# DerEchteKarsten/RayTracer3

Measured on AMD Instinct MI355X. Metric: Mrays/s, higher is better.
Workload: dtype f32

## Files before the change

### raytracer3_amd/csrc/rt3_accel.hip

```cpp
#include <hip/hip_runtime.h>

#include <cmath>
#include <cstring>
#include <algorithm>
#include <chrono>
#include <string>
#include <vector>

#include "rt3_ctx.hpp"

using namespace rt3;

namespace rt3 {

void invalidate_accel(rt3_ctx* c) { c->accel.built = false; }
void mark_accel_stale(rt3_ctx* c) {
    if (c->accel.built) c->accel.stale = true;
}
int check_accel_current(rt3_ctx* c, const char* unbuilt) {
    if (!c || !c->accel.built) return fail(c, RT3_E_STATE, unbuilt);
    if (c->accel.stale) return fail(c, RT3_E_STATE, "vertices were updated since the acceleration structure was built: rt3_accel_refit or rt3_accel_build first");
    return RT3_OK;
}
std::pair<const rt3_instance*, size_t> placements(const rt3_ctx* c, rt3_instance& whole) {
// ... 432 lines not shown
            if (from[q] >= 0) {
                const TlMesh& om = tl.meshes[from[q]];
                meshes[q].n_nodes = om.n_nodes;
                meshes[q].depth = om.depth;
                memcpy(meshes[q].box, om.box, sizeof(om.box));
            } else {
                rc = tl_build_mesh(c, meshes[q], &built[q]);
                tl.n_built++;
            }
        }
        uint64_t nodes_total = head, tris_total = 0;
        for (auto& m : meshes) {
            m.node_off = (uint32_t)nodes_total;
            m.tri_off = (uint32_t)tris_total;
            nodes_total += m.n_nodes;
            tris_total += m.n_tris;
        }
        if (rc == RT3_OK && (nodes_total >= (1ull << 29) || tris_total > (1ull << 28)))
            rc = fail(c, RT3_E_UNSUPPORTED, "instance mode 1: the bottom trees exceed the 28-bit references");
        DevBuf<float4> nodes, tris;
        hipError_t e = hipSuccess;
        if (rc == RT3_OK) {
            e = nodes.alloc_bytes((size_t)nodes_total * 64);
            if (e == hipSuccess) e = tris.alloc_bytes((size_t)tris_total * 48 + 128);
            if (e == hipSuccess) e = hipMemsetAsync((char*)tris.get() + (size_t)tris_total * 48, 0, 128, c->stream);
            for (size_t q = 0; e == hipSuccess && q < meshes.size(); q++) {
                const TlMesh& m = meshes[q];
                if (from[q] >= 0) {
                    const TlMesh& om = tl.meshes[from[q]];
                    tlas_rebase_nodes(c->stream, c->accel.bvh.nodes.get() + 4 * (size_t)om.node_off, nodes.get() + 4 * (size_t)m.node_off, m.n_nodes, om.node_off,
                                      m.node_off, om.tri_off, m.tri_off);
                    e = hipMemcpyAsync(tris.get() + 3 * (size_t)m.tri_off, c->accel.bvh.tris.get() + 3 * (size_t)om.tri_off, (size_t)m.n_tris * 48, hipMemcpyDeviceToDevice,
                                       c->stream);
                } else {
                    tlas_rebase_nodes(c->stream, built[q].nodes.get(), nodes.get() + 4 * (size_t)m.node_off, m.n_nodes, 0u, m.node_off, 0u, m.tri_off);
                    e = hipMemcpyAsync(tris.get() + 3 * (size_t)m.tri_off, built[q].tris.get(), (size_t)m.n_tris * 48, hipMemcpyDeviceToDevice, c->stream);
                }
            }
            if (e == hipSuccess) e = hipGetLastError();
            if (e == hipSuccess) e = hipStreamSynchronize(c->stream);
            if (e != hipSuccess) rc = fail(c, RT3_E_HIP, std::string("two-level: bottom trees: ") + hipGetErrorString(e));
        }
        if (rc != RT3_OK) {
            free_accel(c);
            return rc;
        }
        c->accel.bvh.nodes = std::move(nodes);
        c->accel.bvh.tris = std::move(tris);
        tl.meshes = meshes;
        tl.head = head;
        tl.gen = c->scene.content_gen;
        tl.n_alloc_nodes = (uint32_t)nodes_total;
        tl.valid = true;
    }
    tl.inst = std::move(ii);
    tl.n_placed = n_ne;
    tl.top_cap = top_cap;
    return tl_records_and_top(c);
}
// ... 63 lines not shown
            return rc;
        }
    }
    if (int r = accel_finish(c, out_handle)) return r;
    c->prof.stats.accel_build_ms = std::chrono::duration<double, std::milli>(std::chrono::steady_clock::now() - t_build0).count();
    return RT3_OK;
}
int rt3_accel_info(rt3_ctx* c, uint32_t* n_nodes, uint32_t* n_tris, uint32_t* max_depth, uint32_t* node_bytes) {
    if (!c || !c->accel.built) return fail(c, RT3_E_STATE, "no acceleration structure built");
    if (n_nodes) *n_nodes = c->accel.bvh.n_nodes;
    if (n_tris) *n_tris = c->accel.bvh.n_tris;
    if (max_depth) *max_depth = c->accel.bvh.max_depth;
    if (node_bytes) *node_bytes = c->accel.bvh.node_bytes;
    return RT3_OK;
}
int rt3_accel_levels(rt3_ctx* c, uint32_t* n_meshes, uint32_t* n_meshes_built, uint32_t* n_top_nodes, uint64_t* accel_bytes) {
    if (!c || !c->accel.built) return fail(c, RT3_E_STATE, "no acceleration structure built");
    const bool two = c->accel.bvh.layout == kLayoutTwoLevel;
    if (n_meshes) *n_meshes = two ? c->accel.tl.n_meshes : 0u;
    if (n_meshes_built) *n_meshes_built = two ? c->accel.tl.n_built : 0u;
    if (n_top_nodes) *n_top_nodes = two ? c->accel.tl.n_top : 0u;
    if (accel_bytes) {
        const uint64_t nodes = !c->accel.bvh.nodes ? 0u : (two ? (uint64_t)c->accel.tl.n_alloc_nodes * 64u : (uint64_t)c->accel.bvh.n_nodes * c->accel.bvh.node_bytes);
        *accel_bytes = nodes + (!c->accel.bvh.tris ? 0u : (uint64_t)c->accel.bvh.n_tris * 48u) + (uint64_t)c->accel.bvh.n_top * 64u;
    }
    return RT3_OK;
}
int rt3_accel_download(rt3_ctx* c, void* nodes, size_t nodes_bytes, void* tris, size_t tris_bytes) {
    if (int r = check_accel_current(c, "no acceleration structure built")) return r;
    if (c->accel.bvh.layout == kLayoutTwoLevel) return fail(c, RT3_E_UNSUPPORTED, "accel_download: not for the two-level structure (RT3_OPT_INSTANCE_MODE 1)");
    if (nodes) {
        if (nodes_bytes != (size_t)c->accel.bvh.n_nodes * c->accel.bvh.node_bytes) return fail(c, RT3_E_INVALID, "nodes_bytes mismatch");
        if (nodes_bytes) HIPC(c, hipMemcpy(nodes, c->accel.bvh.nodes.get(), nodes_bytes, hipMemcpyDeviceToHost));
    }
    if (tris) {
        if (tris_bytes != (size_t)c->accel.bvh.n_tris * 48) return fail(c, RT3_E_INVALID, "tris_bytes mismatch");
        if (tris_bytes) HIPC(c, hipMemcpy(tris, c->accel.bvh.tris.get(), tris_bytes, hipMemcpyDeviceToHost));
    }
    return RT3_OK;
}
int rt3_accel_import(rt3_ctx* c, const void* nodes, size_t nodes_bytes, const void* tris, size_t tris_bytes) {
    if (!c || !nodes || !tris) return fail(c, RT3_E_INVALID, "accel_import: NULL argument");
    if (!c->accel.built) return fail(c, RT3_E_STATE, "accel_import: build the scene's own structure first (rt3_accel_build makes the shading records)");
    if (c->accel.bvh.layout == kLayoutTwoLevel) return fail(c, RT3_E_UNSUPPORTED, "accel_import: not for the two-level structure (RT3_OPT_INSTANCE_MODE 1)");
    if (c->accel.bvh.layout != kLayoutWide64Q) return fail(c, RT3_E_UNSUPPORTED, "accel_import: default node layout only");
    if (any_cutoff(c)) return fail(c, RT3_E_UNSUPPORTED, "accel_import: not for a scene with alpha-masked geometry (rt3_scene_set_alpha_cutoffs)");
    if (nodes_bytes == 0 || nodes_bytes % 64 || tris_bytes % 48 || nodes_bytes / 64 > 0x3FFFFFFFull) return fail(c, RT3_E_INVALID, "accel_import: sizes must be multiples of 64 / 48 bytes");
    const uint32_t nn = (uint32_t)(nodes_bytes / 64), nt = (uint32_t)(tris_bytes / 48);
    const uint32_t* w = static_cast<const uint32_t*>(nodes);
    const uint32_t* tw = static_cast<const uint32_t*>(tris);
    for (uint32_t k = 0; k < nt; k++)
        if (tw[12 * (size_t)k + 9] >= c->accel.n_flat_prims) return fail(c, RT3_E_INVALID, "accel_import: triangle record " + std::to_string(k) + " names a primitive the scene does not have");
    std::vector<uint8_t> seen(nn, 0);
    std::vector<std::pair<uint32_t, uint32_t>> st;
    st.emplace_back(0u, 1u);
    seen[0] = 1;
    uint32_t max_level = 1;
    while (!st.empty()) {
        const auto [node, level] = st.back();
        st.pop_back();
        max_level = level > max_level ? level : max_level;
        for (int k = 0; k < 4; k++) {
            const uint32_t ref = w[16 * (size_t)node + 10 + k];
            if (ref == 0xFFFFFFFFu) continue;
            if (ref & 0x80000000u) {
                const uint64_t first = ref & 0x0FFFFFFFu, cnt = ((ref >> 28) & 7u) + 1u;
                if (first + cnt > nt) return fail(c, RT3_E_INVALID, "accel_import: node " + std::to_string(node) + " references triangles beyond the array");
            } else {
                if (ref >= nn || seen[ref]) return fail(c, RT3_E_INVALID, "accel_import: node " + std::to_string(node) + " references a node out of range or reachable twice");
                seen[ref] = 1;
                st.emplace_back(ref, level + 1);
            }
        }
    }
    const uint32_t depth = max_level + 1;
    if (stack_entries(4, depth) > kMaxStack) return fail(c, RT3_E_DEPTH, "accel_import: the tree is deeper than the traversal stack supports");
    HIPC(c, hipSetDevice(c->device));
    HIPC(c, hipStreamSynchronize(c->stream));
    DevBuf<float4> d_nodes, d_tris;
    HIPC(c, d_nodes.alloc_bytes(nodes_bytes));
    hipError_t e = d_tris.alloc_bytes(tris_bytes + 128);
    if (e == hipSuccess) e = hipMemset(d_tris.get(), 0, tris_bytes + 128);
    if (e == hipSuccess) e = hipMemcpy(d_nodes.get(), nodes, nodes_bytes, hipMemcpyHostToDevice);
    if (e == hipSuccess && tris_bytes) e = hipMemcpy(d_tris.get(), tris, tris_bytes, hipMemcpyHostToDevice);
    if (e != hipSuccess) return fail(c, RT3_E_HIP, std::string("accel_import: ") + hipGetErrorString(e));
    c->accel.bvh.nodes = std::move(d_nodes);
    c->accel.bvh.tris = std::move(d_tris);
    c->accel.bvh.n_nodes = nn;
    c->accel.bvh.n_tris = nt;
    c->accel.bvh.max_depth = depth;
    c->accel.refit_planned = false;
    bump_stamp(c);
    e = lbvh_make_top(c->stream, c->accel.bvh.nodes.get(), nn, c->accel.bvh.top, &c->accel.bvh.n_top);
    if (e != hipSuccess) {
        invalidate_accel(c);
        return fail(c, RT3_E_HIP, std::string("accel_import: top-of-tree copy: ") + hipGetErrorString(e));
    }
    return RT3_OK;
}

struct RefitScratch {
    uint32_t* bounds;
    float *nbox, *tbox;
};
static int refit_scratch(rt3_ctx* c, size_t n_nodes, size_t n_tris, RefitScratch* s) {
    BufLayout plan;
    plan.add(&s->bounds, 6).add(&s->nbox, 6 * n_nodes).add(&s->tbox, 6 * n_tris);
// ... 96 lines not shown
```

### raytracer3_amd/csrc/rt3_internal.hpp

```cpp
#pragma once
#include <hip/hip_runtime.h>
#include <stddef.h>
#include <stdint.h>

#include <vector>

#include "rt3_device.hpp"

#define RT3_FLAG_NEE_SKY 1u
#define RT3_FLAG_BLUENOISE 2u
#define RT3_FLAG_SPECULAR 4u
#define RT3_FLAG_FACEFORWARD 8u
#define RT3_FLAG_PROBE_RADIANCE 16u
#define RT3_FLAG_NEE_EMISSIVE 32u

namespace rt3 {

constexpr int kExtendBlock = 256;
constexpr unsigned kExtendMaxBlocks = 2048;
constexpr int kLayoutBinary64 = 0;
constexpr int kLayoutWide128 = 1;
constexpr int kLayoutWide48Q = 3;
constexpr int kC48Stride = 3;
constexpr int kLayoutWide64Q = 2;
constexpr int kLayoutTwoLevel = 4;
constexpr uint32_t kMaxStack = 64;
constexpr uint32_t kTopCacheNodes = 128;
enum TotalsWord : int {
    kTotExtendNodes = 0,
    kTotExtendTris = 1,
    kTotShadowNodes = 2,
    kTotShadowTris = 3,
    kTotExtendLds = 4,
    kTotShadowLds = 5,
    kTotWords = 6
};

struct ShadeLaunch {
    GConstDev g;
    SceneDev sc;
    const uint32_t* pixels;
    const uint2* pixbn;
    uint32_t npix, width;
    FastDiv npix_div;
    uint32_t s0;
    uint32_t bounce;
    const uint4* gbuffer;
    const float* depth;
// ... 246 lines not shown
};
static_assert(sizeof(MotionPrevDev) == 64, "MotionPrev layout");
struct MotionDev {
    const float* verts;
    const uint32_t *indices, *prim_geom, *first_prim, *geom_slot;
    const FlatGeomDev* geoms;
    const MotionPrevDev* prev;
};
struct MotionLaunch {
    GConstDev g;
    MotionDev m;
    const uint32_t* pixels;
    uint32_t npix, width;
    const float* hits;
    void* out;
    const float4* prev_pos = nullptr;
};
void launch_motion(hipStream_t st, const MotionLaunch& L);
void launch_snapshot_positions(hipStream_t st, const float* verts, uint32_t first, uint32_t n, float4* prev_pos);
constexpr uint32_t kDeformChunk = 1024;
void launch_compare_positions(hipStream_t st, const float* verts, const float4* prev_pos, const uint4* chunks, uint32_t n_chunks, uint32_t* flags);

hipError_t lbvh_make_top(hipStream_t st, const float4* nodes, uint32_t n_nodes, DevBuf<float4>& top, uint32_t* n_top);

}
```

### raytracer3_amd/csrc/rt3_kernels.hip

```cpp
#include <hip/hip_fp16.h>
#include <hip/hip_runtime.h>

#include <type_traits>

#include "rt3_device.hpp"
#include "rt3_internal.hpp"

namespace rt3 {

constexpr int kLdsStack = 12;
constexpr uint32_t kTopFlag = 0x40000000u;
constexpr int kSpill = 64 - kLdsStack;
constexpr uint32_t kMaxSteps = 1u << 20;

constexpr uint32_t kEmptySlot = 0xFFFFFFFFu;
constexpr float kTopPadRel = 2.44140625e-4f;

struct Cand {
    float tn;
    uint32_t ref;
};
__device__ __forceinline__ void cswap(Cand& a, Cand& b) {
    bool sw = b.tn < a.tn;
    float ta = a.tn;
// ... 170 lines not shown
                r.sp = 0;
                r.index = idx;
                r.steps = 0u;
                r.cn = r.ct = r.cl = 0u;
                busy = true;
                const float kMaxF = 3.4028234663852886e38f;
                const bool finite_ray = fabsf(r.o.x) <= kMaxF && fabsf(r.o.y) <= kMaxF && fabsf(r.o.z) <= kMaxF && fabsf(r.d.x) <= kMaxF &&
                                        fabsf(r.d.y) <= kMaxF && fabsf(r.d.z) <= kMaxF;
                if (nodes == nullptr || !finite_ray) {
                    finish(r.index, r.best, 0u, 0u, 0u, r.pay0, r.pay1, r.pay2, r.pay3);
                    busy = false;
                }
            }
            const uint32_t taken = (uint32_t)__popcll(m_idle);
            pool_next = pool_next + taken < pool_end ? pool_next + taken : pool_end;
        }
        if (__ballot(busy) == 0ull && pool_next >= pool_end && queue_empty) break;
        if (busy) {
        const bool is_leaf = (r.cur & 0x80000000u) != 0u;
        const uint32_t first = r.cur & 0x0FFFFFFFu, cnt = ((r.cur >> 28) & 7u) + 1u;
        const bool cached = LAYOUT == kLayoutWide64Q && !is_leaf && (r.cur & kTopFlag) != 0u;
        const bool is_inst = TWO && is_leaf && !tl_bottom;
        const bool is_tri = is_leaf && !is_inst;
        const float4* p = is_tri ? tris + 3 * (size_t)(first + r.leaf_k)
                                 : nodes + (WIDE ? 8 : (C48 ? kC48Stride : 4)) * (size_t)(cached ? 0u : (is_inst ? first : r.cur));
        float4 q0, q1, q2, q3, q4, q5, q6, q7;
        if (LAYOUT == kLayoutWide64Q && cached) {
            const float4* t = top_lds + 4 * (r.cur & 0xFFFFu);
            q0 = t[0];
            q1 = t[1];
            q2 = t[2];
            q3 = t[3];
        } else {
            q0 = p[0];
            q1 = p[1];
            q2 = p[2];
            q3 = C48 ? make_float4(0.0f, 0.0f, 0.0f, 0.0f) : p[3];
        }
        if (WIDE) {
            q4 = p[4];
            q5 = p[5];
            q6 = p[6];
            q7 = p[7];
        }
        if (TWO && is_tri) {
            const float4* pm = nodes + 4 * (size_t)(tl_rec + 1u);
            q4 = pm[0];
// ... 1003 lines not shown
```

### raytracer3_amd/csrc/rt3_lbvh.hip

```cpp
#include <hip/hip_runtime.h>
#include <hipcub/hipcub.hpp>

#include <chrono>
#include <cstdio>
#include <cstdlib>
#include <vector>

#include "rt3_device.hpp"
#include "rt3_internal.hpp"
#include "rt3_bvh_device.hpp"

namespace rt3 {

__global__ void k_prim_geom(const uint32_t* first_prim, uint32_t n_geoms, uint32_t n, uint32_t* prim_geom) {
    for (uint32_t p = blockIdx.x * blockDim.x + threadIdx.x; p < n; p += gridDim.x * blockDim.x) {
        uint32_t lo = 0, hi = n_geoms;
        while (hi - lo > 1u) {
            uint32_t mid = (lo + hi) >> 1;
            if (first_prim[mid] <= p) lo = mid;
            else hi = mid;
        }
        prim_geom[p] = lo;
    }
}
// ... 85 lines not shown

__global__ void k_morton(const float* bmin, const float* bmax, const uint32_t* bounds, uint32_t n, uint64_t* keys, uint32_t* vals) {
    float cmin[3], cext[3];
#pragma unroll
    for (int k = 0; k < 3; k++) {
        cmin[k] = ordered_to_float(bounds[6 + k]);
        cext[k] = ordered_to_float(bounds[9 + k]) - cmin[k];
    }
    for (uint32_t i = blockIdx.x * blockDim.x + threadIdx.x; i < n; i += gridDim.x * blockDim.x) {
        uint32_t q[3];
#pragma unroll
        for (int k = 0; k < 3; k++) {
            float ce = (bmin[3 * (size_t)i + k] + bmax[3 * (size_t)i + k]) * 0.5f;
            float nrm = cext[k] > 0.0f ? (ce - cmin[k]) / cext[k] : 0.0f;
            q[k] = (uint32_t)fmin_sel(nrm * 2097152.0f, 2097151.0f);
        }
        keys[i] = (expand21(q[0]) << 2) | (expand21(q[1]) << 1) | expand21(q[2]);
        vals[i] = i;
    }
}

__global__ void k_leaves(const float* verts, const uint32_t* indices, const FlatGeomDev* geoms, const uint32_t* prim_geom,
                         const uint32_t* first_prim, const uint32_t* sorted_prim, const float* bmin, const float* bmax,
                         const uint32_t* bounds, uint32_t n, float4* tris, float* lmin, float* lmax, const uint2* geom_mask) {
    const float pad = leaf_pad(bounds);
    for (uint32_t k = blockIdx.x * blockDim.x + threadIdx.x; k < n; k += gridDim.x * blockDim.x) {
        uint32_t p = sorted_prim[k];
        V3 a, b, c;
        fetch_triangle(verts, indices, geoms, prim_geom, first_prim, p, a, b, c);
        tris[3 * (size_t)k + 0] = make_float4(a.x, a.y, a.z, b.x);
        tris[3 * (size_t)k + 1] = make_float4(b.y, b.z, c.x, c.y);
        const uint2 mk = geom_mask ? geom_mask[geoms[prim_geom[p]].geom] : make_uint2(0u, 0u);
        tris[3 * (size_t)k + 2] = make_float4(c.z, __uint_as_float(p), __uint_as_float(mk.x), __uint_as_float(mk.y));
#pragma unroll
        for (int j = 0; j < 3; j++) {
            lmin[3 * (size_t)k + j] = bmin[3 * (size_t)p + j] - pad;
            lmax[3 * (size_t)k + j] = bmax[3 * (size_t)p + j] + pad;
        }
    }
}

__device__ __forceinline__ int delta(const uint64_t* codes, int n, int i, int j) {
    if (j < 0 || j >= n) return -1;
    uint64_t a = codes[i], b = codes[j];
    if (a != b) return __clzll((long long)(a ^ b));
    return 64 + __clz((int)((uint32_t)i ^ (uint32_t)j));
}

__global__ void k_hierarchy(const uint64_t* codes, int n, uint32_t* left, uint32_t* right, uint32_t* parent_internal, uint32_t* parent_leaf,
                            uint32_t* range_lo, uint32_t* range_cnt) {
    for (int i = blockIdx.x * blockDim.x + threadIdx.x; i < n - 1; i += gridDim.x * blockDim.x) {
        int d = (delta(codes, n, i, i + 1) - delta(codes, n, i, i - 1)) >= 0 ? 1 : -1;
        int dmin = delta(codes, n, i, i - d);
        int lmax = 2;
        while (delta(codes, n, i, i + lmax * d) > dmin) lmax *= 2;
        int l = 0;
// ... 209 lines not shown
        }
    }
}
__device__ __forceinline__ uint32_t tree_position(uint32_t me_ref, uint32_t parent, const uint32_t* left, const uint32_t* right, const uint32_t* parent_internal,
                                                  const uint32_t* range_cnt) {
    uint32_t pos = 0;
    while (parent != 0xFFFFFFFFu) {
        if (right[parent] == me_ref) {
            const uint32_t l = left[parent];
            pos += (l & 0x80000000u) ? 1u : range_cnt[l];
        }
        me_ref = parent;
        parent = parent_internal[parent];
    }
    return pos;
}
__global__ void k_tree_order(const uint32_t* left, const uint32_t* right, const uint32_t* parent_internal, const uint32_t* parent_leaf, const uint32_t* range_cnt,
                             uint32_t n, uint32_t nn, uint32_t* newpos, uint32_t* range_lo) {
    for (uint32_t t = blockIdx.x * blockDim.x + threadIdx.x; t < n + nn; t += gridDim.x * blockDim.x) {
        if (t < n) newpos[t] = tree_position(0x80000000u | t, parent_leaf[t], left, right, parent_internal, range_cnt);
        else range_lo[t - n] = tree_position(t - n, parent_internal[t - n], left, right, parent_internal, range_cnt);
    }
}
__global__ void k_tree_reorder(const uint32_t* newpos, uint32_t n, uint32_t nn, const float4* tris_in, float4* tris_out, const float* lmin_in, const float* lmax_in,
                               float* lmin_out, float* lmax_out, uint32_t* left, uint32_t* right) {
    for (uint32_t t = blockIdx.x * blockDim.x + threadIdx.x; t < n + nn; t += gridDim.x * blockDim.x) {
        if (t < n) {
            const uint32_t p = newpos[t];
#pragma unroll
            for (int k = 0; k < 3; k++) tris_out[3 * (size_t)p + k] = tris_in[3 * (size_t)t + k];
#pragma unroll
            for (int j = 0; j < 3; j++) {
                lmin_out[3 * (size_t)p + j] = lmin_in[3 * (size_t)t + j];
                lmax_out[3 * (size_t)p + j] = lmax_in[3 * (size_t)t + j];
            }
        } else {
            const uint32_t i = t - n, l = left[i], r = right[i];
            if (l & 0x80000000u) left[i] = 0x80000000u | newpos[l & 0x7FFFFFFFu];
            if (r & 0x80000000u) right[i] = 0x80000000u | newpos[r & 0x7FFFFFFFu];
        }
    }
}

__device__ __forceinline__ uint32_t gather_slots(uint32_t i, const uint32_t* left, const uint32_t* right, const uint32_t* live,
                                                 const float* nbox, const uint32_t* dk, int wide, int collapse, uint32_t sl[4]) {
    uint32_t ns = 0;
    if (wide && collapse == 2) {
        uint32_t sn[8], sm[8];
        int sp = 0;
        const uint32_t k4 = dk[i] & 3u;
        sl[0] = sl[1] = sl[2] = sl[3] = 0xFFFFFFFFu;
        sn[sp] = right[i]; sm[sp++] = 4u - k4;
        sn[sp] = left[i]; sm[sp++] = k4;
// ... 163 lines not shown
__global__ void k_top_cache(const float4* __restrict__ nodes, uint32_t n_nodes, uint32_t* __restrict__ top_words , uint32_t* __restrict__ n_top_out) {
    if (blockIdx.x != 0 || threadIdx.x != 0) return;
    uint32_t queue[kTopCacheNodes];
    uint32_t head = 0, tail = 0;
    if (n_nodes) queue[tail++] = 0u;
    while (head < tail) {
        const uint32_t node = queue[head];
        const uint32_t* src = reinterpret_cast<const uint32_t*>(nodes + 4 * (size_t)node);
        uint32_t* dst = top_words + 16 * (size_t)head;
        for (int k = 0; k < 16; k++) dst[k] = src[k];
        for (int k = 0; k < 4; k++) {
            const uint32_t ref = src[10 + k];
            if (ref == 0xFFFFFFFFu || (ref & 0x80000000u)) continue;
            if (tail < kTopCacheNodes) {
                dst[10 + k] = 0x40000000u | tail;
                queue[tail++] = ref;
            }
        }
        head++;
    }
    *n_top_out = tail;
}

hipError_t lbvh_make_top(hipStream_t st, const float4* nodes, uint32_t n_nodes, DevBuf<float4>& top, uint32_t* n_top) {
    *n_top = 0;
    if (!top) {
        hipError_t e = top.alloc_bytes((size_t)kTopCacheNodes * 64);
        if (e != hipSuccess) return e;
    }
    DevBuf<uint32_t> d_ntop;
    hipError_t e = d_ntop.alloc_bytes(4);
    if (e != hipSuccess) return e;
    hipLaunchKernelGGL(k_top_cache, dim3(1), dim3(1), 0, st, nodes, n_nodes, (uint32_t*)top.get(), d_ntop.get());
    e = hipMemcpyAsync(n_top, d_ntop.get(), 4, hipMemcpyDeviceToHost, st);
    if (e == hipSuccess) e = hipStreamSynchronize(st);
    return e;
}

__global__ void k_single(const float* lmin, const float* lmax, int wide, int quant, float4* nodes) {
    const float inf = INFINITY;
    if (wide && quant) {
        float qmn[4][3], qmx[4][3];
        uint32_t qref[4] = {0x80000000u, 0, 0, 0};
        for (int j = 0; j < 3; j++) {
            qmn[0][j] = lmin[j];
            qmx[0][j] = lmax[j];
// ... 64 lines not shown
    const bool dp = collapse == 2;
    out->node_bytes = (wide && !quant) ? 128u : (quant == 2 ? 16u * kC48Stride : 64u);
    out->layout = !wide ? kLayoutBinary64 : (quant == 2 ? kLayoutWide48Q : (quant ? kLayoutWide64Q : kLayoutWide128));
    if (n == 0) return hipSuccess;
    const uint32_t nn = n > 1 ? n - 1 : 1;
    LbvhScratch s = {};
    {
        BufLayout plan;
        RT3_TRY(plan_scratch(st, n, quant, collapse, sah_top != 0, wide && quant == 1, plan, &s));
        RT3_TRY(scratch.grow_bytes(plan.bytes()));
        RT3_TRY(plan.carve(scratch));
        if (getenv("RT3_TRACE_BUILD"))
            fprintf(stderr, "rt3 build: %u triangles, scratch %zu bytes (radix sort %zu, scan %zu)\n", n, plan.bytes(), s.sort_bytes, s.scan_bytes);
    }
    const unsigned grid = (unsigned)(((uint64_t)n + 255) / 256 > 4096 ? 4096 : ((uint64_t)n + 255) / 256);
    uint32_t init_bounds[12];
    uint32_t tail[2] = {0, 0};
    for (int k = 0; k < 3; k++) {
        init_bounds[k] = 0xFFFFFFFFu;
        init_bounds[3 + k] = 0u;
        init_bounds[6 + k] = 0xFFFFFFFFu;
        init_bounds[9 + k] = 0u;
    }
    RT3_TRY(out->tris.alloc_bytes((size_t)n * 48 + 128));
    RT3_TRY(hipMemsetAsync((char*)out->tris.get() + (size_t)n * 48, 0, 128, st));
    RT3_TRY(hipMemcpyAsync(s.bounds, init_bounds, sizeof(init_bounds), hipMemcpyHostToDevice, st));
    RT3_TRY(hipMemsetAsync(s.arrive, 0, (size_t)nn * 4, st));
    RT3_TRY(hipMemsetAsync(s.levels, 0, 4, st));
    hipLaunchKernelGGL(k_prim_bounds, dim3(grid > 512 ? 512 : grid), dim3(256), 0, st, t.verts, t.indices, t.geoms, t.prim_geom, t.first_prim, n, s.bmin, s.bmax, s.bounds);
    hipLaunchKernelGGL(k_morton, dim3(grid), dim3(256), 0, st, s.bmin, s.bmax, s.bounds, n, s.keys_in, s.vals_in);
    RT3_TRY(hipcub::DeviceRadixSort::SortPairs(s.sort_tmp, s.sort_bytes, s.keys_in, s.keys_out, s.vals_in, s.vals_out, (int)n, 0, 63, st));
    hipLaunchKernelGGL(k_leaves, dim3(grid), dim3(256), 0, st, t.verts, t.indices, t.geoms, t.prim_geom, t.first_prim, s.vals_out, s.bmin, s.bmax, s.bounds, n,
                       s.tris_dp ? s.tris_dp : (s.tris_morton ? s.tris_morton : out->tris.get()), s.lmin, s.lmax, geom_mask);
    if (n == 1) {
        RT3_TRY(out->nodes.alloc_bytes(out->node_bytes));
        hipLaunchKernelGGL(k_single, dim3(1), dim3(1), 0, st, s.lmin, s.lmax, wide, quant, out->nodes.get());
        out->n_nodes = 1;
        out->max_depth = 2;
        RT3_TRY(hipGetLastError());
        RT3_TRY(hipStreamSynchronize(st));
    } else {
        hipLaunchKernelGGL(k_hierarchy, dim3(grid), dim3(256), 0, st, s.keys_out, (int)n, s.left, s.right, s.pint, s.pleaf, s.rlo, s.rcnt);
        const uint32_t T_sah = dp ? sah_top : (sah_top > leaf_max ? sah_top : leaf_max);
        const bool lite = sah_top && T_sah <= 64;
        if (lite) hipLaunchKernelGGL(k_refit_clusters, dim3(grid), dim3(256), 0, st, s.rlo, s.rcnt, s.lmin, s.lmax, nn, T_sah, s.nbox);
        else hipLaunchKernelGGL(k_refit, dim3(grid), dim3(256), 0, st, s.left, s.right, s.pint, s.pleaf, s.lmin, s.lmax, n, s.nbox, s.arrive);
        if (sah_top) {
            bool relinked = false;
            const auto t0 = std::chrono::steady_clock::now();
            RT3_TRY(sah_top_relink_gpu(st, nn, s.left, s.right, s.rcnt, s.pint, s.pleaf, s.lmin, s.lmax, s.nbox, T_sah, s.sah, &relinked));
            if (!relinked && lite) {
                RT3_TRY(hipMemsetAsync(s.arrive, 0, (size_t)nn * 4, st));
                hipLaunchKernelGGL(k_refit, dim3(grid), dim3(256), 0, st, s.left, s.right, s.pint, s.pleaf, s.lmin, s.lmax, n, s.nbox, s.arrive);
            }
            if (getenv("RT3_TRACE_BUILD")) {
                RT3_TRY(hipStreamSynchronize(st));
                fprintf(stderr, "rt3 build: device SAH top (incl. GPU LBVH drain) %.2f ms\n",
                        std::chrono::duration<double, std::milli>(std::chrono::steady_clock::now() - t0).count());
            }
        }
        const auto t3 = std::chrono::steady_clock::now();
        if (dp) {
            RT3_TRY(hipMemsetAsync(s.arrive, 0, (size_t)nn * 4, st));
            hipLaunchKernelGGL(k_dp_up, dim3(grid), dim3(256), 0, st, s.left, s.right, s.pint, s.pleaf, s.lmin, s.lmax, s.nbox, n, leaf_max, s.rcnt, s.dc, s.dk,
                               s.live, s.arrive);
            const unsigned g3 = (unsigned)(((uint64_t)n + nn + 255) / 256 > 4096 ? 4096 : ((uint64_t)n + nn + 255) / 256);
            hipLaunchKernelGGL(k_tree_order, dim3(g3), dim3(256), 0, st, s.left, s.right, s.pint, s.pleaf, s.rcnt, n, nn, s.newpos, s.rlo);
            float4* tris_to = quant == 2 ? s.tris_morton : out->tris.get();
            hipLaunchKernelGGL(k_tree_reorder, dim3(g3), dim3(256), 0, st, s.newpos, n, nn, s.tris_dp, tris_to, s.lmin, s.lmax, s.lmin2, s.lmax2, s.left, s.right);
            s.lmin = s.lmin2;
            s.lmax = s.lmax2;
        } else {
            hipLaunchKernelGGL(k_live_flags, dim3(grid), dim3(256), 0, st, s.rcnt, nn, leaf_max, s.live);
        }
        if (collapse) {
            const uint32_t root = 0, one = 1;
            const size_t n_cnt = (size_t)nn + 18;
            RT3_TRY(hipMemsetAsync(s.keep, 0, (size_t)nn * 4, st));
            RT3_TRY(hipMemsetAsync(s.fr_n, 0, n_cnt * 4, st));
            RT3_TRY(hipMemcpyAsync(s.fr_a, &root, 4, hipMemcpyHostToDevice, st));
            RT3_TRY(hipMemcpyAsync(s.fr_n, &one, 4, hipMemcpyHostToDevice, st));
            const unsigned g2 = (unsigned)((nn + 255) / 256 > 1024 ? 1024 : (nn + 255) / 256);
            uint32_t level = 0, last = 1, wide_levels = 0;
            while (last > 0 && level + 16 < n_cnt) {
                for (int burst = 0; burst < 16; burst++, level++) {
                    hipLaunchKernelGGL(k_wide_level, dim3(g2), dim3(256), 0, st, s.left, s.right, s.live, s.nbox, s.dk, collapse, s.fr_a, s.fr_n + level, s.keep,
                                       s.fr_b, s.fr_n + level + 1);
                    std::swap(s.fr_a, s.fr_b);
                }
                RT3_TRY(hipMemcpyAsync(&last, s.fr_n + level, 4, hipMemcpyDeviceToHost, st));
                RT3_TRY(hipStreamSynchronize(st));
            }
// ... 41 lines not shown
```

### raytracer3_amd/csrc/rt3_refit.hip

```cpp
#include <hip/hip_runtime.h>

#include "rt3_bvh_device.hpp"
#include "rt3_internal.hpp"

namespace rt3 {

namespace {

__global__ void k_plan_root(uint32_t root, uint32_t* order, uint32_t* level_count) {
    order[0] = root;
    level_count[0] = 1u;
}

__global__ void k_plan_level(const float4* __restrict__ nodes, uint32_t level, uint32_t cap, uint32_t* order, uint32_t* level_count) {
    uint32_t start = 0;
    for (uint32_t l = 0; l < level; l++) start += level_count[l];
    const uint32_t n = level_count[level], next = start + n;
    for (uint32_t f = blockIdx.x * blockDim.x + threadIdx.x; f < n && start + f < cap; f += gridDim.x * blockDim.x) {
        const uint32_t* w = reinterpret_cast<const uint32_t*>(nodes + 4 * (size_t)order[start + f]);
        for (int k = 0; k < 4; k++) {
            const uint32_t ref = w[10 + k];
            if (ref == 0xFFFFFFFFu || (ref & 0x80000000u)) continue;
            const uint32_t at = next + atomicAdd(&level_count[level + 1], 1u);
            if (at < cap) order[at] = ref;
// ... 24 lines not shown
    }
    __shared__ uint32_t s_b[6];
    if (threadIdx.x < 6) s_b[threadIdx.x] = threadIdx.x < 3 ? 0xFFFFFFFFu : 0u;
    __syncthreads();
    if ((threadIdx.x & 63) == 0) {
#pragma unroll
        for (int k = 0; k < 3; k++) {
            atomicMin(&s_b[k], float_to_ordered(lo[k]));
            atomicMax(&s_b[3 + k], float_to_ordered(hi[k]));
        }
    }
    __syncthreads();
    if (threadIdx.x < 6) {
        if (threadIdx.x < 3) atomicMin(&bounds[threadIdx.x], s_b[threadIdx.x]);
        else atomicMax(&bounds[threadIdx.x], s_b[threadIdx.x]);
    }
}

__global__ void k_refit_tris(const float* verts, const uint32_t* indices, const FlatGeomDev* geoms, const uint32_t* prim_geom, const uint32_t* first_prim,
                             const uint32_t* bounds, uint32_t first, uint32_t n, float4* tris, float* tbox) {
    const float pad = leaf_pad(bounds);
    for (uint32_t i = blockIdx.x * blockDim.x + threadIdx.x; i < n; i += gridDim.x * blockDim.x) {
        const size_t k = (size_t)first + i;
        const uint32_t p = __float_as_uint(tris[3 * k + 2].y);
        V3 a, b, c;
        fetch_triangle(verts, indices, geoms, prim_geom, first_prim, p, a, b, c);
        tris[3 * k + 0] = make_float4(a.x, a.y, a.z, b.x);
        tris[3 * k + 1] = make_float4(b.y, b.z, c.x, c.y);
        tris[3 * k + 2] = make_float4(c.z, __uint_as_float(p), tris[3 * k + 2].z, tris[3 * k + 2].w);
        tbox[6 * k + 0] = fmin_sel(a.x, fmin_sel(b.x, c.x)) - pad;
        tbox[6 * k + 1] = fmin_sel(a.y, fmin_sel(b.y, c.y)) - pad;
        tbox[6 * k + 2] = fmin_sel(a.z, fmin_sel(b.z, c.z)) - pad;
        tbox[6 * k + 3] = fmax_sel(a.x, fmax_sel(b.x, c.x)) + pad;
        tbox[6 * k + 4] = fmax_sel(a.y, fmax_sel(b.y, c.y)) + pad;
        tbox[6 * k + 5] = fmax_sel(a.z, fmax_sel(b.z, c.z)) + pad;
    }
}

__global__ void k_refit_level(const uint32_t* __restrict__ order, uint32_t start, uint32_t n, const float* __restrict__ tbox, float* nbox, float4* nodes) {
    for (uint32_t f = blockIdx.x * blockDim.x + threadIdx.x; f < n; f += gridDim.x * blockDim.x) {
        const uint32_t node = order[start + f];
        float4* nd = nodes + 4 * (size_t)node;
        uint32_t ref[4];
        {
            const float4 q2 = nd[2], q3 = nd[3];
            ref[0] = __float_as_uint(q2.z);
            ref[1] = __float_as_uint(q2.w);
            ref[2] = __float_as_uint(q3.x);
            ref[3] = __float_as_uint(q3.y);
        }
        float mn[4][3], mx[4][3], box[6] = {INFINITY, INFINITY, INFINITY, -INFINITY, -INFINITY, -INFINITY};
        uint32_t qref[4] = {0, 0, 0, 0}, ns = 0;
// ... 85 lines not shown
```

### raytracer3_amd/csrc/rt3_tlas.hip

```cpp
#include <hip/hip_runtime.h>

#include "rt3_device.hpp"
#include "rt3_internal.hpp"

namespace rt3 {

__global__ void k_tlas_rebase(const float4* __restrict__ src, float4* __restrict__ dst, uint32_t n, uint32_t node_from, uint32_t node_to,
                              uint32_t tri_from, uint32_t tri_to) {
    for (uint32_t i = blockIdx.x * blockDim.x + threadIdx.x; i < n; i += gridDim.x * blockDim.x) {
        float4 q0 = src[4 * (size_t)i], q1 = src[4 * (size_t)i + 1], q2 = src[4 * (size_t)i + 2], q3 = src[4 * (size_t)i + 3];
        uint32_t r[4] = {__float_as_uint(q2.z), __float_as_uint(q2.w), __float_as_uint(q3.x), __float_as_uint(q3.y)};
        for (int k = 0; k < 4; k++) {
            if (r[k] == 0xFFFFFFFFu) continue;
            if (r[k] & 0x80000000u) r[k] = (r[k] & 0xF0000000u) | ((r[k] & 0x0FFFFFFFu) - tri_from + tri_to);
            else r[k] = r[k] - node_from + node_to;
        }
        q2.z = __uint_as_float(r[0]);
        q2.w = __uint_as_float(r[1]);
        q3.x = __uint_as_float(r[2]);
        q3.y = __uint_as_float(r[3]);
        dst[4 * (size_t)i] = q0;
        dst[4 * (size_t)i + 1] = q1;
        dst[4 * (size_t)i + 2] = q2;
        dst[4 * (size_t)i + 3] = q3;
// ... 13 lines not shown
            const float* c = v == 1 ? b + 3 : b;
            o[0] = c[0];
            o[1] = c[1];
            o[2] = c[2];
            for (int k = 3; k < 8; k++) o[k] = 0.0f;
            o[3 + 2] = 1.0f;
            indices[3 * (size_t)i + v] = 3u * i + (uint32_t)v;
        }
    }
}
void tlas_box_tris(hipStream_t st, const float* boxes, uint32_t n, float* verts, uint32_t* indices) {
    if (n == 0) return;
    const unsigned grid = (n + 255) / 256 > 1024 ? 1024 : (n + 255) / 256;
    hipLaunchKernelGGL(k_tlas_box_tris, dim3(grid), dim3(256), 0, st, boxes, n, verts, indices);
}

__global__ void k_tlas_emit_top(const float4* __restrict__ top_nodes, uint32_t n, const float4* __restrict__ top_tris, uint32_t rec_base,
                                float4* __restrict__ dst) {
    for (uint32_t i = blockIdx.x * blockDim.x + threadIdx.x; i < n; i += gridDim.x * blockDim.x) {
        float4 q2 = top_nodes[4 * (size_t)i + 2], q3 = top_nodes[4 * (size_t)i + 3];
        uint32_t r[4] = {__float_as_uint(q2.z), __float_as_uint(q2.w), __float_as_uint(q3.x), __float_as_uint(q3.y)};
        for (int k = 0; k < 4; k++) {
            if (r[k] == 0xFFFFFFFFu || !(r[k] & 0x80000000u)) continue;
            const uint32_t slot = __float_as_uint(top_tris[3 * (size_t)(r[k] & 0x0FFFFFFFu) + 2].y);
            r[k] = 0x80000000u | (rec_base + 2u * slot);
        }
        q2.z = __uint_as_float(r[0]);
        q2.w = __uint_as_float(r[1]);
        q3.x = __uint_as_float(r[2]);
        q3.y = __uint_as_float(r[3]);
        dst[4 * (size_t)i] = top_nodes[4 * (size_t)i];
        dst[4 * (size_t)i + 1] = top_nodes[4 * (size_t)i + 1];
        dst[4 * (size_t)i + 2] = q2;
        dst[4 * (size_t)i + 3] = q3;
    }
}
void tlas_emit_top(hipStream_t st, const float4* top_nodes, uint32_t n_nodes, const float4* top_tris, uint32_t rec_base, float4* dst) {
    if (n_nodes == 0) return;
    const unsigned grid = (n_nodes + 255) / 256 > 1024 ? 1024 : (n_nodes + 255) / 256;
    hipLaunchKernelGGL(k_tlas_emit_top, dim3(grid), dim3(256), 0, st, top_nodes, n_nodes, top_tris, rec_base, dst);
}

}
```

Baseline: 7558.

## Pad triangle records to 64-byte stride for wide quantized layouts

Changes the triangle record stride from 48 to 64 bytes (4 float4) for the wide-64Q and two-level layouts, so each triangle fetch in traversal is aligned to a 64-byte line. The build, reorder, refit, TLAS and import/export paths are updated, and a restride kernel converts to and from the packed 48-byte format at the API boundary. The aim is fewer cache-line splits on triangle loads during traversal, paid for with a third more triangle memory and bandwidth.

```diff
diff --git a/raytracer3_amd/csrc/rt3_accel.hip b/raytracer3_amd/csrc/rt3_accel.hip
--- a/raytracer3_amd/csrc/rt3_accel.hip
+++ b/raytracer3_amd/csrc/rt3_accel.hip
@@ -478,19 +478,20 @@
         hipError_t e = hipSuccess;
         if (rc == RT3_OK) {
             e = nodes.alloc_bytes((size_t)nodes_total * 64);
-            if (e == hipSuccess) e = tris.alloc_bytes((size_t)tris_total * 48 + 128);
-            if (e == hipSuccess) e = hipMemsetAsync((char*)tris.get() + (size_t)tris_total * 48, 0, 128, c->stream);
+            constexpr size_t ts = tri_stride(kLayoutTwoLevel), tri_bytes = 16 * ts;
+            if (e == hipSuccess) e = tris.alloc_bytes((size_t)tris_total * tri_bytes + kTriSlackBytes);
+            if (e == hipSuccess) e = hipMemsetAsync((char*)tris.get() + (size_t)tris_total * tri_bytes, 0, kTriSlackBytes, c->stream);
             for (size_t q = 0; e == hipSuccess && q < meshes.size(); q++) {
                 const TlMesh& m = meshes[q];
                 if (from[q] >= 0) {
                     const TlMesh& om = tl.meshes[from[q]];
                     tlas_rebase_nodes(c->stream, c->accel.bvh.nodes.get() + 4 * (size_t)om.node_off, nodes.get() + 4 * (size_t)m.node_off, m.n_nodes, om.node_off,
                                       m.node_off, om.tri_off, m.tri_off);
-                    e = hipMemcpyAsync(tris.get() + 3 * (size_t)m.tri_off, c->accel.bvh.tris.get() + 3 * (size_t)om.tri_off, (size_t)m.n_tris * 48, hipMemcpyDeviceToDevice,
-                                       c->stream);
+                    e = hipMemcpyAsync(tris.get() + ts * (size_t)m.tri_off, c->accel.bvh.tris.get() + ts * (size_t)om.tri_off, (size_t)m.n_tris * tri_bytes,
+                                       hipMemcpyDeviceToDevice, c->stream);
                 } else {
                     tlas_rebase_nodes(c->stream, built[q].nodes.get(), nodes.get() + 4 * (size_t)m.node_off, m.n_nodes, 0u, m.node_off, 0u, m.tri_off);
-                    e = hipMemcpyAsync(tris.get() + 3 * (size_t)m.tri_off, built[q].tris.get(), (size_t)m.n_tris * 48, hipMemcpyDeviceToDevice, c->stream);
+                    e = hipMemcpyAsync(tris.get() + ts * (size_t)m.tri_off, built[q].tris.get(), (size_t)m.n_tris * tri_bytes, hipMemcpyDeviceToDevice, c->stream);
                 }
             }
             if (e == hipSuccess) e = hipGetLastError();
@@ -600,7 +601,7 @@
     if (n_top_nodes) *n_top_nodes = two ? c->accel.tl.n_top : 0u;
     if (accel_bytes) {
         const uint64_t nodes = !c->accel.bvh.nodes ? 0u : (two ? (uint64_t)c->accel.tl.n_alloc_nodes * 64u : (uint64_t)c->accel.bvh.n_nodes * c->accel.bvh.node_bytes);
-        *accel_bytes = nodes + (!c->accel.bvh.tris ? 0u : (uint64_t)c->accel.bvh.n_tris * 48u) + (uint64_t)c->accel.bvh.n_top * 64u;
+        *accel_bytes = nodes + (!c->accel.bvh.tris ? 0u : (uint64_t)c->accel.bvh.n_tris * 16u * tri_stride(c->accel.bvh.layout)) + (uint64_t)c->accel.bvh.n_top * 64u;
     }
     return RT3_OK;
 }
@@ -613,7 +614,17 @@
     }
     if (tris) {
         if (tris_bytes != (size_t)c->accel.bvh.n_tris * 48) return fail(c, RT3_E_INVALID, "tris_bytes mismatch");
-        if (tris_bytes) HIPC(c, hipMemcpy(tris, c->accel.bvh.tris.get(), tris_bytes, hipMemcpyDeviceToHost));
+        const uint32_t ts = tri_stride(c->accel.bvh.layout);
+        if (tris_bytes && ts == kTriStridePacked) {
+            HIPC(c, hipMemcpy(tris, c->accel.bvh.tris.get(), tris_bytes, hipMemcpyDeviceToHost));
+        } else if (tris_bytes) {
+            DevBuf<float4> packed;
+            HIPC(c, packed.alloc_bytes(tris_bytes));
+            launch_tri_restride(c->stream, c->accel.bvh.tris.get(), ts, packed.get(), kTriStridePacked, c->accel.bvh.n_tris);
+            HIPC(c, hipGetLastError());
+            HIPC(c, hipMemcpyAsync(tris, packed.get(), tris_bytes, hipMemcpyDeviceToHost, c->stream));
+            HIPC(c, hipStreamSynchronize(c->stream));
+        }
     }
     return RT3_OK;
 }
@@ -657,10 +668,18 @@
     HIPC(c, hipStreamSynchronize(c->stream));
     DevBuf<float4> d_nodes, d_tris;
     HIPC(c, d_nodes.alloc_bytes(nodes_bytes));
-    hipError_t e = d_tris.alloc_bytes(tris_bytes + 128);
-    if (e == hipSuccess) e = hipMemset(d_tris.get(), 0, tris_bytes + 128);
+    constexpr uint32_t ts = tri_stride(kLayoutWide64Q);
+    DevBuf<float4> packed;
+    hipError_t e = d_tris.alloc_bytes((size_t)nt * 16 * ts + kTriSlackBytes);
+    if (e == hipSuccess) e = hipMemset((char*)d_tris.get() + (size_t)nt * 16 * ts, 0, kTriSlackBytes);
     if (e == hipSuccess) e = hipMemcpy(d_nodes.get(), nodes, nodes_bytes, hipMemcpyHostToDevice);
-    if (e == hipSuccess && tris_bytes) e = hipMemcpy(d_tris.get(), tris, tris_bytes, hipMemcpyHostToDevice);
+    if (e == hipSuccess && nt) e = packed.alloc_bytes(tris_bytes);
+    if (e == hipSuccess && nt) e = hipMemcpy(packed.get(), tris, tris_bytes, hipMemcpyHostToDevice);
+    if (e == hipSuccess && nt) {
+        launch_tri_restride(c->stream, packed.get(), kTriStridePacked, d_tris.get(), ts, nt);
+        e = hipGetLastError();
+        if (e == hipSuccess) e = hipStreamSynchronize(c->stream);
+    }
     if (e != hipSuccess) return fail(c, RT3_E_HIP, std::string("accel_import: ") + hipGetErrorString(e));
     c->accel.bvh.nodes = std::move(d_nodes);
     c->accel.bvh.tris = std::move(d_tris);
diff --git a/raytracer3_amd/csrc/rt3_internal.hpp b/raytracer3_amd/csrc/rt3_internal.hpp
--- a/raytracer3_amd/csrc/rt3_internal.hpp
+++ b/raytracer3_amd/csrc/rt3_internal.hpp
@@ -24,6 +24,10 @@
 constexpr int kC48Stride = 3;
 constexpr int kLayoutWide64Q = 2;
 constexpr int kLayoutTwoLevel = 4;
+constexpr uint32_t kTriStridePacked = 3;
+constexpr uint32_t kTriStride64Q = 4;
+constexpr uint32_t tri_stride(int layout) { return layout == kLayoutWide64Q || layout == kLayoutTwoLevel ? kTriStride64Q : kTriStridePacked; }
+constexpr size_t kTriSlackBytes = 128;
 constexpr uint32_t kMaxStack = 64;
 constexpr uint32_t kTopCacheNodes = 128;
 enum TotalsWord : int {
@@ -316,5 +320,6 @@
 void launch_compare_positions(hipStream_t st, const float* verts, const float4* prev_pos, const uint4* chunks, uint32_t n_chunks, uint32_t* flags);
 
 hipError_t lbvh_make_top(hipStream_t st, const float4* nodes, uint32_t n_nodes, DevBuf<float4>& top, uint32_t* n_top);
+void launch_tri_restride(hipStream_t st, const float4* src, uint32_t src_stride, float4* dst, uint32_t dst_stride, uint32_t n);
 
 }
diff --git a/raytracer3_amd/csrc/rt3_kernels.hip b/raytracer3_amd/csrc/rt3_kernels.hip
--- a/raytracer3_amd/csrc/rt3_kernels.hip
+++ b/raytracer3_amd/csrc/rt3_kernels.hip
@@ -216,7 +216,7 @@
         const bool cached = LAYOUT == kLayoutWide64Q && !is_leaf && (r.cur & kTopFlag) != 0u;
         const bool is_inst = TWO && is_leaf && !tl_bottom;
         const bool is_tri = is_leaf && !is_inst;
-        const float4* p = is_tri ? tris + 3 * (size_t)(first + r.leaf_k)
+        const float4* p = is_tri ? tris + tri_stride(LAYOUT) * (size_t)(first + r.leaf_k)
                                  : nodes + (WIDE ? 8 : (C48 ? kC48Stride : 4)) * (size_t)(cached ? 0u : (is_inst ? first : r.cur));
         float4 q0, q1, q2, q3, q4, q5, q6, q7;
         if (LAYOUT == kLayoutWide64Q && cached) {
diff --git a/raytracer3_amd/csrc/rt3_lbvh.hip b/raytracer3_amd/csrc/rt3_lbvh.hip
--- a/raytracer3_amd/csrc/rt3_lbvh.hip
+++ b/raytracer3_amd/csrc/rt3_lbvh.hip
@@ -131,16 +131,18 @@
 
 __global__ void k_leaves(const float* verts, const uint32_t* indices, const FlatGeomDev* geoms, const uint32_t* prim_geom,
                          const uint32_t* first_prim, const uint32_t* sorted_prim, const float* bmin, const float* bmax,
-                         const uint32_t* bounds, uint32_t n, float4* tris, float* lmin, float* lmax, const uint2* geom_mask) {
+                         const uint32_t* bounds, uint32_t n, float4* tris, uint32_t stride, float* lmin, float* lmax, const uint2* geom_mask) {
     const float pad = leaf_pad(bounds);
     for (uint32_t k = blockIdx.x * blockDim.x + threadIdx.x; k < n; k += gridDim.x * blockDim.x) {
         uint32_t p = sorted_prim[k];
         V3 a, b, c;
         fetch_triangle(verts, indices, geoms, prim_geom, first_prim, p, a, b, c);
-        tris[3 * (size_t)k + 0] = make_float4(a.x, a.y, a.z, b.x);
-        tris[3 * (size_t)k + 1] = make_float4(b.y, b.z, c.x, c.y);
+        float4* rec = tris + stride * (size_t)k;
+        rec[0] = make_float4(a.x, a.y, a.z, b.x);
+        rec[1] = make_float4(b.y, b.z, c.x, c.y);
         const uint2 mk = geom_mask ? geom_mask[geoms[prim_geom[p]].geom] : make_uint2(0u, 0u);
-        tris[3 * (size_t)k + 2] = make_float4(c.z, __uint_as_float(p), __uint_as_float(mk.x), __uint_as_float(mk.y));
+        rec[2] = make_float4(c.z, __uint_as_float(p), __uint_as_float(mk.x), __uint_as_float(mk.y));
+        for (uint32_t j = kTriStridePacked; j < stride; j++) rec[j] = make_float4(0.0f, 0.0f, 0.0f, 0.0f);
 #pragma unroll
         for (int j = 0; j < 3; j++) {
             lmin[3 * (size_t)k + j] = bmin[3 * (size_t)p + j] - pad;
@@ -396,13 +398,14 @@
         else range_lo[t - n] = tree_position(t - n, parent_internal[t - n], left, right, parent_internal, range_cnt);
     }
 }
-__global__ void k_tree_reorder(const uint32_t* newpos, uint32_t n, uint32_t nn, const float4* tris_in, float4* tris_out, const float* lmin_in, const float* lmax_in,
+__global__ void k_tree_reorder(const uint32_t* newpos, uint32_t n, uint32_t nn, const float4* tris_in, float4* tris_out, uint32_t stride, const float* lmin_in, const float* lmax_in,
                                float* lmin_out, float* lmax_out, uint32_t* left, uint32_t* right) {
     for (uint32_t t = blockIdx.x * blockDim.x + threadIdx.x; t < n + nn; t += gridDim.x * blockDim.x) {
         if (t < n) {
             const uint32_t p = newpos[t];
 #pragma unroll
-            for (int k = 0; k < 3; k++) tris_out[3 * (size_t)p + k] = tris_in[3 * (size_t)t + k];
+            for (int k = 0; k < 3; k++) tris_out[stride * (size_t)p + k] = tris_in[3 * (size_t)t + k];
+            for (uint32_t k = kTriStridePacked; k < stride; k++) tris_out[stride * (size_t)p + k] = make_float4(0.0f, 0.0f, 0.0f, 0.0f);
 #pragma unroll
             for (int j = 0; j < 3; j++) {
                 lmin_out[3 * (size_t)p + j] = lmin_in[3 * (size_t)t + j];
@@ -612,6 +615,19 @@
     *n_top_out = tail;
 }
 
+__global__ void k_tri_restride(const float4* __restrict__ src, uint32_t src_stride, float4* __restrict__ dst, uint32_t dst_stride, uint32_t n) {
+    for (uint32_t i = blockIdx.x * blockDim.x + threadIdx.x; i < n; i += gridDim.x * blockDim.x) {
+#pragma unroll
+        for (uint32_t k = 0; k < kTriStridePacked; k++) dst[dst_stride * (size_t)i + k] = src[src_stride * (size_t)i + k];
+        for (uint32_t k = kTriStridePacked; k < dst_stride; k++) dst[dst_stride * (size_t)i + k] = make_float4(0.0f, 0.0f, 0.0f, 0.0f);
+    }
+}
+void launch_tri_restride(hipStream_t st, const float4* src, uint32_t src_stride, float4* dst, uint32_t dst_stride, uint32_t n) {
+    if (n == 0) return;
+    const unsigned grid = (n + 255) / 256 > 4096 ? 4096 : (n + 255) / 256;
+    hipLaunchKernelGGL(k_tri_restride, dim3(grid), dim3(256), 0, st, src, src_stride, dst, dst_stride, n);
+}
+
 hipError_t lbvh_make_top(hipStream_t st, const float4* nodes, uint32_t n_nodes, DevBuf<float4>& top, uint32_t* n_top) {
     *n_top = 0;
     if (!top) {
@@ -722,8 +738,9 @@
         init_bounds[6 + k] = 0xFFFFFFFFu;
         init_bounds[9 + k] = 0u;
     }
-    RT3_TRY(out->tris.alloc_bytes((size_t)n * 48 + 128));
-    RT3_TRY(hipMemsetAsync((char*)out->tris.get() + (size_t)n * 48, 0, 128, st));
+    const uint32_t stride = tri_stride(out->layout);
+    RT3_TRY(out->tris.alloc_bytes((size_t)n * 16 * stride + kTriSlackBytes));
+    RT3_TRY(hipMemsetAsync((char*)out->tris.get() + (size_t)n * 16 * stride, 0, kTriSlackBytes, st));
     RT3_TRY(hipMemcpyAsync(s.bounds, init_bounds, sizeof(init_bounds), hipMemcpyHostToDevice, st));
     RT3_TRY(hipMemsetAsync(s.arrive, 0, (size_t)nn * 4, st));
     RT3_TRY(hipMemsetAsync(s.levels, 0, 4, st));
@@ -731,7 +748,8 @@
     hipLaunchKernelGGL(k_morton, dim3(grid), dim3(256), 0, st, s.bmin, s.bmax, s.bounds, n, s.keys_in, s.vals_in);
     RT3_TRY(hipcub::DeviceRadixSort::SortPairs(s.sort_tmp, s.sort_bytes, s.keys_in, s.keys_out, s.vals_in, s.vals_out, (int)n, 0, 63, st));
     hipLaunchKernelGGL(k_leaves, dim3(grid), dim3(256), 0, st, t.verts, t.indices, t.geoms, t.prim_geom, t.first_prim, s.vals_out, s.bmin, s.bmax, s.bounds, n,
-                       s.tris_dp ? s.tris_dp : (s.tris_morton ? s.tris_morton : out->tris.get()), s.lmin, s.lmax, geom_mask);
+                       s.tris_dp ? s.tris_dp : (s.tris_morton ? s.tris_morton : out->tris.get()), (s.tris_dp || s.tris_morton) ? kTriStridePacked : stride, s.lmin,
+                       s.lmax, geom_mask);
     if (n == 1) {
         RT3_TRY(out->nodes.alloc_bytes(out->node_bytes));
         hipLaunchKernelGGL(k_single, dim3(1), dim3(1), 0, st, s.lmin, s.lmax, wide, quant, out->nodes.get());
@@ -767,7 +785,8 @@
             const unsigned g3 = (unsigned)(((uint64_t)n + nn + 255) / 256 > 4096 ? 4096 : ((uint64_t)n + nn + 255) / 256);
             hipLaunchKernelGGL(k_tree_order, dim3(g3), dim3(256), 0, st, s.left, s.right, s.pint, s.pleaf, s.rcnt, n, nn, s.newpos, s.rlo);
             float4* tris_to = quant == 2 ? s.tris_morton : out->tris.get();
-            hipLaunchKernelGGL(k_tree_reorder, dim3(g3), dim3(256), 0, st, s.newpos, n, nn, s.tris_dp, tris_to, s.lmin, s.lmax, s.lmin2, s.lmax2, s.left, s.right);
+            hipLaunchKernelGGL(k_tree_reorder, dim3(g3), dim3(256), 0, st, s.newpos, n, nn, s.tris_dp, tris_to, quant == 2 ? kTriStridePacked : stride, s.lmin, s.lmax, s.lmin2,
+                               s.lmax2, s.left, s.right);
             s.lmin = s.lmin2;
             s.lmax = s.lmax2;
         } else {
diff --git a/raytracer3_amd/csrc/rt3_refit.hip b/raytracer3_amd/csrc/rt3_refit.hip
--- a/raytracer3_amd/csrc/rt3_refit.hip
+++ b/raytracer3_amd/csrc/rt3_refit.hip
@@ -70,12 +70,13 @@
     const float pad = leaf_pad(bounds);
     for (uint32_t i = blockIdx.x * blockDim.x + threadIdx.x; i < n; i += gridDim.x * blockDim.x) {
         const size_t k = (size_t)first + i;
-        const uint32_t p = __float_as_uint(tris[3 * k + 2].y);
+        float4* rec = tris + tri_stride(kLayoutWide64Q) * k;
+        const uint32_t p = __float_as_uint(rec[2].y);
         V3 a, b, c;
         fetch_triangle(verts, indices, geoms, prim_geom, first_prim, p, a, b, c);
-        tris[3 * k + 0] = make_float4(a.x, a.y, a.z, b.x);
-        tris[3 * k + 1] = make_float4(b.y, b.z, c.x, c.y);
-        tris[3 * k + 2] = make_float4(c.z, __uint_as_float(p), tris[3 * k + 2].z, tris[3 * k + 2].w);
+        rec[0] = make_float4(a.x, a.y, a.z, b.x);
+        rec[1] = make_float4(b.y, b.z, c.x, c.y);
+        rec[2] = make_float4(c.z, __uint_as_float(p), rec[2].z, rec[2].w);
         tbox[6 * k + 0] = fmin_sel(a.x, fmin_sel(b.x, c.x)) - pad;
         tbox[6 * k + 1] = fmin_sel(a.y, fmin_sel(b.y, c.y)) - pad;
         tbox[6 * k + 2] = fmin_sel(a.z, fmin_sel(b.z, c.z)) - pad;
diff --git a/raytracer3_amd/csrc/rt3_tlas.hip b/raytracer3_amd/csrc/rt3_tlas.hip
--- a/raytracer3_amd/csrc/rt3_tlas.hip
+++ b/raytracer3_amd/csrc/rt3_tlas.hip
@@ -59,7 +59,7 @@
         uint32_t r[4] = {__float_as_uint(q2.z), __float_as_uint(q2.w), __float_as_uint(q3.x), __float_as_uint(q3.y)};
         for (int k = 0; k < 4; k++) {
             if (r[k] == 0xFFFFFFFFu || !(r[k] & 0x80000000u)) continue;
-            const uint32_t slot = __float_as_uint(top_tris[3 * (size_t)(r[k] & 0x0FFFFFFFu) + 2].y);
+            const uint32_t slot = __float_as_uint(top_tris[tri_stride(kLayoutWide64Q) * (size_t)(r[k] & 0x0FFFFFFFu) + 2].y);
             r[k] = 0x80000000u | (rec_base + 2u * slot);
         }
         q2.z = __uint_as_float(r[0]);
```

Measured after the change: 7598, median of 6. About the same (+0.5%).
